# toposware/schnorr-sig

Hardware: AMD Instinct MI355X
Metric: Schnorr verifications/sec, 2^20-sig batch, 1/2/4/8 MI355X; bit-exact vs CPU (higher is better)
Workload: dtype u64

## Files before the change

### __graft_entry__.py

```python
import os
import subprocess
import sys

ROOT = os.path.dirname(os.path.abspath(__file__))
CSRC = os.path.join(ROOT, "schnorr-sig_amd", "csrc")
LIB = os.path.join(CSRC, "libschnorr_sig_amd.so")


def _sources():
    return sorted(f for f in os.listdir(CSRC) if f.endswith((".hip", ".hpp", ".hpp", ".inc")))


STAMP = LIB + ".srchash"


def _source_hash(deps):
    import hashlib
    h = hashlib.sha256()
    for d in sorted(deps):
        h.update(os.path.basename(d).encode() + b"\0")
        with open(d, "rb") as fh:
            h.update(fh.read())
        h.update(b"\0")
    return h.hexdigest()


HIPCC_FLAGS = ["-O3", "--offload-arch=gfx950", "-std=c++17", "-fPIC"]


def _file_sha256(path):
    import hashlib
    h = hashlib.sha256()
    with open(path, "rb") as fh:
        for blk in iter(lambda: fh.read(1 << 20), b""):
            h.update(blk)
    return h.hexdigest()


_TOOLCHAIN = []


def _toolchain():
    if not _TOOLCHAIN:
        try:
            _TOOLCHAIN.append(subprocess.run(["hipcc", "--version"], capture_output=True, text=True, timeout=60).stdout.strip())
        except Exception:
            _TOOLCHAIN.append(None)
    return _TOOLCHAIN[0]


def _stamp(deps):
    return {"sources": _source_hash(deps), "flags": " ".join(HIPCC_FLAGS), "hipcc": _toolchain()}


def _stale(target, deps):
    import json
    if not os.path.exists(target) or not os.path.exists(STAMP):
        return True
    try:
        with open(STAMP) as fh:
            st = json.load(fh)
    except ValueError:
        return True
    want = _stamp(deps)
    if want["hipcc"] is None:
        want.pop("hipcc")
    return any(st.get(k) != v for k, v in want.items()) or st.get("library_sha256") != _file_sha256(target)


def build(force=False):
    params_inc = os.path.join(ROOT, "schnorr-sig_amd", "params", "params_default.inc")
    if not os.path.exists(params_inc):
        subprocess.check_call([sys.executable, os.path.join(ROOT, "schnorr-sig_amd", "params", "gen_params.py")])
    deps = [os.path.join(CSRC, s) for s in _sources()] + [params_inc, os.path.join(ROOT, "include", "schnorr_sig_amd.h")]
    if force or _stale(LIB, deps):
        if _toolchain() is None:
            raise RuntimeError("the HIP library is missing or stale and there is no hipcc on this host to rebuild it")
        objs, procs = [], []
        for unit in ("ssa_api", "ssa_msm", "ssa_sign"):
            objs.append(unit + ".o")
            procs.append(subprocess.Popen(["hipcc"] + HIPCC_FLAGS + ["-c", "-cuid=" + unit, "-o", unit + ".o",
                                           unit + ".hip"], cwd=CSRC))
        for pr in procs:
            if pr.wait() != 0:
                raise subprocess.CalledProcessError(pr.returncode, pr.args)
        subprocess.check_call(["hipcc", "--offload-arch=gfx950", "-fPIC", "-shared", "-o", os.path.basename(LIB)] + objs,
                              cwd=CSRC)
        objs = [os.path.join(CSRC, o) for o in objs]
        for obj in objs:
            os.remove(obj)
        import json
        st = _stamp(deps)
        st["library_sha256"] = _file_sha256(LIB)
        with open(STAMP, "w") as fh:
            json.dump(st, fh, indent=1)
    subprocess.check_call(["make", "-s", "-C", os.path.join(ROOT, "oracle")])
    if ROOT not in sys.path:
        sys.path.insert(0, ROOT)
    import schnorr_sig_amd


def smoke():
    import numpy as np
    if ROOT not in sys.path:
        sys.path.insert(0, ROOT)
    sys.path.insert(0, os.path.join(ROOT, "oracle"))
    import schnorr_sig_amd as ssa
    from oracle import Oracle

    n = 256
    rng = np.random.default_rng(0x5C4E0222)
    sks = rng.integers(0, 256, size=(n, 32), dtype=np.uint8)
    sks[:, 31] &= 0x3F
    nonces = rng.integers(0, 256, size=(n, 32), dtype=np.uint8)
    nonces[:, 31] &= 0x3F
    msgs = rng.integers(0, 256, size=(n, 80), dtype=np.uint8)
    eng = ssa.Engine(0)
    pks, sigs = eng.keygen_sign_many(sks, nonces, msgs)
    orc = Oracle()
    pks_o, sigs_o = orc.keygen_sign_many(sks[:16], nonces[:16], msgs[:16])
    assert (pks[:16] == pks_o).all() and (sigs[:16] == sigs_o).all(), "GPU keygen/sign != oracle"
    sigs[3, 49] ^= 1
    msgs[7, 0] ^= 1
    pks[11] = pks[12]
    status, nfail = eng.verify_many(sigs, pks, msgs, check_torsion=True)
    expect = orc.verify_many(sigs, pks, msgs, check_torsion=True)
    assert (status == expect).all(), "GPU status vector != oracle"
    assert nfail == int((expect != 0).sum()) == 3
    print("smoke ok: %d signatures, %d rejected as expected" % (n, nfail))


if __name__ == "__main__":
    build()
    if len(sys.argv) > 1 and sys.argv[1] == "smoke":
        smoke()
```

### schnorr-sig_amd/csrc/curve.hpp

```cpp
#pragma once
#include "fp6.hpp"

namespace ssa {

struct jac {
    fp6 X, Y, Z;
};
struct aff {
    fp6 x, y;
};

SSA_DEV jac jac_identity() {
    jac r;
    r.X = f6_one();
    r.Y = f6_one();
    r.Z = f6_zero();
    return r;
}
SSA_DEV bool jac_is_identity(const jac &p) { return f6_is_zero(p.Z); }

#ifdef SSA_DBL_PLAIN
SSA_DEV jac jac_dbl(const jac &p) {
    fp6 XX = f6_sqr(p.X);
    fp6 YY = f6_sqr(p.Y);
    fp6 YYYY = f6_sqr(YY);
    fp6 ZZ = f6_sqr(p.Z);
    fp6 t = f6_add(p.X, YY);
    fp6 S = f6_dbl(f6_sub(f6_sub(f6_sqr(t), XX), YYYY));
    fp6 M = f6_add(f6_add(f6_dbl(XX), XX), f6_sqr(ZZ));
    jac r;
    r.X = f6_sub(f6_sqr(M), f6_dbl(S));
    fp6 y8 = f6_dbl(f6_dbl(f6_dbl(YYYY)));
    r.Y = f6_sub(f6_mul(M, f6_sub(S, r.X)), y8);
    fp6 yz = f6_add(p.Y, p.Z);
    r.Z = f6_sub(f6_sub(f6_sqr(yz), YY), ZZ);
    return r;
}
#else
SSA_DEV jac jac_dbl(const jac &p) {
#ifdef SSA_DBL_INLINE
    const fp6 XX = f6_sqr_inl(p.X);
    const fp6 YY = f6_sqr_inl(p.Y);
    const fp6 YYYY = f6_sqr_inl(YY);
    const fp6 ZZ = f6_sqr_inl(p.Z);
#else
    const fp6 XX = f6_sqr(p.X);
    const fp6 YY = f6_sqr(p.Y);
    const fp6 YYYY = f6_sqr(YY);
    const fp6 ZZ = f6_sqr(p.Z);
#endif
    const fp6 Sh = f6_sqr_sub2(f6_add(p.X, YY), XX, YYYY);
    const fp6 M = f6_sqr_add3x(ZZ, XX);
    jac r;
    r.X = f6_sqr_sub4x(M, Sh);
    r.Y = f6_mul_sub8x(M, f6_sub(f6_dbl(Sh), r.X), YYYY);
    r.Z = f6_sqr_sub2(f6_add(p.Y, p.Z), YY, ZZ);
    return r;
}
#endif

#if defined(SSA_F6_ASM) && !defined(SSA_NO_JAC_ASM)
#define SSA_JAC_ASM 1
#ifdef SSA_JAC_ASM_INC
#include SSA_JAC_ASM_INC
#else
#include "jac_asm.inc"
#endif
#endif
SSA_DEV jac jac_dbl_n(jac p, u32 n) {
    if (n == 0) return p;
#ifdef SSA_JAC_ASM
    jac_dbl_n_asm(p.X.c, p.Y.c, p.Z.c, n);
    return p;
#else
#pragma unroll 1
    for (u32 d = 0; d < n; d++) p = jac_dbl(p);
    return p;
#endif
}

SSA_FN void jac_dbl_cold(jac *__restrict__ r, const jac *__restrict__ p) { *r = jac_dbl(*p); }

SSA_DEV jac jac_madd(const jac &p, const aff &q) {
#ifdef SSA_MADD_PLAIN
    fp6 Z1Z1 = f6_sqr(p.Z);
    fp6 U2 = f6_mul(q.x, Z1Z1);
    fp6 S2 = f6_mul(f6_mul(q.y, p.Z), Z1Z1);
    fp6 H = f6_sub(U2, p.X);
    fp6 R = f6_sub(S2, p.Y);
#else
    const fp6 Z1Z1 = f6_sqr(p.Z);
    u64 zz7[6];
    f6_mul_prescale(Z1Z1, zz7);
    const fp6 H = f6_mul_subx_pre(q.x, Z1Z1, zz7, p.X);
    const fp6 R = f6_mul_subx_pre(f6_mul(q.y, p.Z), Z1Z1, zz7, p.Y);
#endif
    const bool p_inf = f6_is_zero(p.Z);
    const bool q_inf = f6_is_zero(q.x) && f6_is_zero(q.y);
    const bool h0 = f6_is_zero(H);
    const bool r0 = f6_is_zero(R);
    if (!p_inf && !q_inf && h0 && r0) {
#ifndef SSA_MADD_COLD_DBL
        return jac_dbl(p);
#else
        jac d;
        jac_dbl_cold(&d, &p);
        return d;
#endif
    }
    fp6 HH = f6_sqr(H);
    fp6 HHH = f6_mul(H, HH);
    fp6 V = f6_mul(p.X, HH);
    jac r;
#ifdef SSA_MADD_PLAIN
    r.X = f6_sub(f6_sub(f6_sqr(R), HHH), f6_dbl(V));
    r.Y = f6_sub(f6_mul(R, f6_sub(V, r.X)), f6_mul(p.Y, HHH));
#else
    r.X = f6_sqr_subx_sub2y(R, HHH, V);
    r.Y = f6_mul2_add(R, f6_sub(V, r.X), f6_neg(p.Y), HHH);
#endif
    r.Z = f6_mul(p.Z, H);
    if (p_inf) {
        r.X = q.x;
        r.Y = q.y;
        r.Z = q_inf ? f6_zero() : f6_one();
    }
    if (q_inf && !p_inf) r = p;
    return r;
}

SSA_DEV jac jac_madd_fast(const jac &p, const aff &q) {
#ifdef SSA_JAC_ASM
    jac r = p;
    if (jac_madd_asm(r.X.c, r.Y.c, r.Z.c, q.x.c, q.y.c)) return r;
    return jac_madd(r, q);
#else
    return jac_madd(p, q);
#endif
}

SSA_DEV jac jac_add(const jac &p, const jac &q) {
    fp6 Z1Z1 = f6_sqr(p.Z);
    fp6 Z2Z2 = f6_sqr(q.Z);
    fp6 U1 = f6_mul(p.X, Z2Z2);
    fp6 U2 = f6_mul(q.X, Z1Z1);
    fp6 S1 = f6_mul(f6_mul(p.Y, q.Z), Z2Z2);
    fp6 S2 = f6_mul(f6_mul(q.Y, p.Z), Z1Z1);
    fp6 H = f6_sub(U2, U1);
    fp6 R = f6_sub(S2, S1);
    const bool p_inf = f6_is_zero(p.Z);
    const bool q_inf = f6_is_zero(q.Z);
    if (!p_inf && !q_inf && f6_is_zero(H) && f6_is_zero(R)) {
#ifndef SSA_MADD_COLD_DBL
        return jac_dbl(p);
#else
        jac d;
        jac_dbl_cold(&d, &p);
        return d;
#endif
    }
    fp6 HH = f6_sqr(H);
    fp6 HHH = f6_mul(H, HH);
    fp6 V = f6_mul(U1, HH);
    jac r;
    r.X = f6_sub(f6_sub(f6_sqr(R), HHH), f6_dbl(V));
    r.Y = f6_sub(f6_mul(R, f6_sub(V, r.X)), f6_mul(S1, HHH));
    r.Z = f6_mul(f6_mul(p.Z, q.Z), H);
    if (p_inf) r = q;
    if (q_inf && !p_inf) r = p;
    return r;
}

SSA_DEV jac jac_neg_if(const jac &p, bool neg) {
    jac r = p;
    fp6 ny = f6_neg(p.Y);
    r.Y = f6_select(neg, p.Y, ny);
    return r;
}

SSA_DEV jac jac_from_aff(const aff &a) {
    jac r;
    r.X = a.x;
    r.Y = a.y;
    r.Z = f6_one();
    return r;
}

SSA_DEV aff jac_to_aff(const jac &p) {
    aff r;
    if (f6_is_zero(p.Z)) {
        r.x = f6_zero();
        r.y = f6_zero();
        return r;
    }
    fp6 zi = f6_inv(p.Z);
    fp6 zi2 = f6_sqr(zi);
    r.x = f6_canon(f6_mul(p.X, zi2));
    r.y = f6_canon(f6_mul(p.Y, f6_mul(zi, zi2)));
    return r;
}

struct sc256 {
    u64 w[4];
};
SSA_DEV u64 sc_q_limb(int i) {
    switch (i) {
        case 0: return 0xd443623eaed4accfULL;
        case 1: return 0x327aa72330157722ULL;
        case 2: return 0x563fbf0f990a37b5ULL;
        default: return 0x7af2599b3b3f22d0ULL;
    }
}
#define SC_Q(i) sc_q_limb(i)

SSA_DEV bool sc_geq_q(const sc256 &a) {
    bool ge = true;
#pragma unroll
    for (int i = 0; i < 4; i++) {
        if (a.w[i] > SC_Q(i)) ge = true;
// ... 95 lines not shown
```

### schnorr-sig_amd/csrc/ssa_kernels.hpp

```cpp
#pragma once
#include "curve.hpp"
#include "fp3.hpp"
#include "rescue.hpp"

namespace ssa {

struct GtabGeom {
    u32 bits, count;
};
constexpr int GW_BITS_MAX = 24, GW_BITS_MIN = 16;
__host__ __device__ inline u32 gtab_windows(u32 bits) { return (255u + bits) / bits; }
__host__ __device__ inline size_t gtab_entries(u32 bits) { return (size_t)gtab_windows(bits) << bits; }
__host__ __device__ inline size_t gbase_entries(u32 bits) { return ((size_t)gtab_windows(bits) * 2) << (bits / 2); }
__host__ __device__ inline u64 gtab_header(u32 bits) { return (u64)bits | ((u64)gtab_windows(bits) << 8); }
SSA_DEV GtabGeom gtab_geom(const u64 *__restrict__ gtab) {
    const u32 v = (u32)__builtin_amdgcn_readfirstlane((int)(u32)gtab[0]);
    GtabGeom g;
    g.bits = v & 0xffu;
    g.count = (v >> 8) & 0xffu;
    return g;
}
constexpr int PTAB_ENTRIES = 16;
constexpr int PTAB_ENTRY_U64 = 32, PTAB_Z = 16, PTAB_C = 22;
constexpr int PTAB_NEG = 16, PTAB_NY = PTAB_NEG + 6;
// ... 209 lines not shown
SSA_DEV void st_row(u64 *__restrict__ row, const jac &p) {
    st_f6(row, p.X);
    st_f6(row + 6, p.Y);
    st_f6(row + PTAB_Z, p.Z);
}
SSA_DEV jac ld_row(const u64 *__restrict__ row) {
    jac p;
    p.X = ld_f6(row);
    p.Y = ld_f6(row + 6);
    p.Z = ld_f6(row + PTAB_Z);
    return p;
}

SSA_FN void tab_dbl(u64 *__restrict__ dst, const u64 *__restrict__ src) { st_row(dst, jac_dbl(ld_row(src))); }
SSA_FN void tab_madd(u64 *__restrict__ dst, const u64 *__restrict__ src, const u64 *__restrict__ paff) {
    st_row(dst, jac_madd(ld_row(src), ld_aff(paff)));
}

SSA_DEV fp6 aff_dbl_num(const fp6 &x) {
    const fp6 xx = f6_sqr(x);
    fp6 n = f6_add(f6_dbl(xx), xx);
    n.c[0] = fp_add(n.c[0], 1ull);
    return n;
}
SSA_DEV aff aff_from_slope(const fp6 &l, const fp6 &x1, const fp6 &y1, const fp6 &x2) {
    aff r;
    r.x = f6_sub(f6_sub(f6_sqr(l), x1), x2);
    r.y = f6_sub(f6_mul(l, f6_sub(x1, r.x)), y1);
    return r;
}
SSA_DEV void st_tab_entry(u64 *__restrict__ row, const aff &a) {
    st_aff(row, a);
    st_f6(row + PTAB_NEG, a.x);
    st_f6(row + PTAB_NY, f6_neg(a.y));
}
SSA_DEV bool build_ptab_affine_upper(u64 *__restrict__ tab) {
    constexpr int R = PTAB_ENTRY_U64;
    const aff p8 = ld_aff(tab + 7 * R);
    fp6 c = f6_one();
#pragma unroll 1
    for (int m = 9; m <= 16; m++) {
        const aff b = ld_aff(tab + (((m & 1) ? m - 8 : m / 2) - 1) * R);
        const fp6 d = (m & 1) ? f6_sub(p8.x, b.x) : f6_dbl(b.y);
        st_f6(tab + (m - 1) * R + PTAB_Z, d);
        c = f6_mul(c, d);
        st_f6(tab + (m - 1) * R + PTAB_C, c);
    }
    if (f6_is_zero(c)) return false;
    fp6 inv = f6_inv(c);
#pragma unroll 1
    for (int m = 16; m >= 9; m--) {
        fp6 di = inv;
        if (m > 9) di = f6_mul(inv, ld_f6(tab + (m - 2) * R + PTAB_C));
        inv = f6_mul(inv, ld_f6(tab + (m - 1) * R + PTAB_Z));
        const aff b = ld_aff(tab + (((m & 1) ? m - 8 : m / 2) - 1) * R);
        aff r;
        if (m & 1) r = aff_from_slope(f6_mul(f6_sub(p8.y, b.y), di), b.x, b.y, p8.x);
        else r = aff_from_slope(f6_mul(aff_dbl_num(b.x), di), b.x, b.y, b.x);
        st_tab_entry(tab + (m - 1) * R, r);
    }
    return true;
}

SSA_DEV bool build_ptab_affine(u64 *__restrict__ tab, const aff &p) {
    constexpr int R = PTAB_ENTRY_U64;
    const fp6 d2 = f6_dbl(p.y);
    if (f6_is_zero(d2)) return false;
    const aff p2 = aff_from_slope(f6_mul(aff_dbl_num(p.x), f6_inv(d2)), p.x, p.y, p.x);
    const fp6 a3 = f6_sub(p2.x, p.x), a4 = f6_dbl(p2.y);
    const fp6 t34 = f6_mul(a3, a4);
    if (f6_is_zero(t34)) return false;
    const fp6 i34 = f6_inv(t34);
    const aff p3 = aff_from_slope(f6_mul(f6_sub(p2.y, p.y), f6_mul(i34, a4)), p.x, p.y, p2.x);
    const aff p4 = aff_from_slope(f6_mul(aff_dbl_num(p2.x), f6_mul(i34, a3)), p2.x, p2.y, p2.x);
    const fp6 a5 = f6_sub(p4.x, p.x), a6 = f6_dbl(p3.y), a7 = f6_sub(p4.x, p3.x), a8 = f6_dbl(p4.y);
    const fp6 t56 = f6_mul(a5, a6), t567 = f6_mul(t56, a7), t5678 = f6_mul(t567, a8);
    if (f6_is_zero(t5678)) return false;
    fp6 inv = f6_inv(t5678);
    const fp6 i8 = f6_mul(inv, t567);
    inv = f6_mul(inv, a8);
    const fp6 i7 = f6_mul(inv, t56);
    inv = f6_mul(inv, a7);
    const fp6 i6 = f6_mul(inv, a5), i5 = f6_mul(inv, a6);
    st_tab_entry(tab, p);
    st_tab_entry(tab + 1 * R, p2);
    st_tab_entry(tab + 2 * R, p3);
    st_tab_entry(tab + 3 * R, p4);
    st_tab_entry(tab + 4 * R, aff_from_slope(f6_mul(f6_sub(p4.y, p.y), i5), p.x, p.y, p4.x));
    st_tab_entry(tab + 5 * R, aff_from_slope(f6_mul(aff_dbl_num(p3.x), i6), p3.x, p3.y, p3.x));
    st_tab_entry(tab + 6 * R, aff_from_slope(f6_mul(f6_sub(p4.y, p3.y), i7), p3.x, p3.y, p4.x));
    st_tab_entry(tab + 7 * R, aff_from_slope(f6_mul(aff_dbl_num(p4.x), i8), p4.x, p4.y, p4.x));
    return build_ptab_affine_upper(tab);
}

SSA_DEV void build_ptab(u64 *__restrict__ tab, const aff &p, bool p_inf) {
    constexpr int R = PTAB_ENTRY_U64;
    if (p_inf) {
        aff z;
        z.x = f6_zero();
        z.y = f6_zero();
#pragma unroll 1
        for (int e = 0; e < PTAB_ENTRIES; e++) st_tab_entry(tab + e * R, z);
        return;
    }
#ifndef SSA_PTAB_JACOBIAN_ONLY
    if (build_ptab_affine(tab, p)) return;
#endif
    st_row(tab, jac_from_aff(p));
    tab_dbl(tab + 1 * R, tab);
    tab_madd(tab + 2 * R, tab + 1 * R, tab);
    tab_dbl(tab + 3 * R, tab + 1 * R);
    tab_madd(tab + 4 * R, tab + 3 * R, tab);
    tab_dbl(tab + 5 * R, tab + 2 * R);
    tab_madd(tab + 6 * R, tab + 5 * R, tab);
    tab_dbl(tab + 7 * R, tab + 3 * R);
#pragma unroll 1
    for (int m = 9; m <= 16; m++) {
        if (m & 1) tab_madd(tab + (m - 1) * R, tab + (m - 2) * R, tab);
        else tab_dbl(tab + (m - 1) * R, tab + (m / 2 - 1) * R);
    }
    fp6 c = f6_one();
#pragma unroll 1
    for (int e = 1; e < PTAB_ENTRIES; e++) {
        fp6 z = ld_f6(tab + e * R + PTAB_Z);
        if (f6_is_zero(z)) z = f6_one();
        c = f6_mul(c, z);
        st_f6(tab + e * R + PTAB_C, c);
    }
    fp6 inv = f6_inv(c);
#pragma unroll 1
    for (int e = PTAB_ENTRIES - 1; e >= 1; e--) {
        fp6 z = ld_f6(tab + e * R + PTAB_Z);
        const bool zero = f6_is_zero(z);
        if (zero) z = f6_one();
        fp6 zinv = inv;
        if (e > 1) zinv = f6_mul(inv, ld_f6(tab + (e - 1) * R + PTAB_C));
        inv = f6_mul(inv, z);
        const fp6 zi2 = f6_sqr(zinv);
        aff a;
        a.x = f6_mul(ld_f6(tab + e * R), zi2);
        a.y = f6_mul(ld_f6(tab + e * R + 6), f6_mul(zi2, zinv));
        if (zero) {
            a.x = f6_zero();
            a.y = f6_zero();
        }
        st_tab_entry(tab + e * R, a);
    }
    st_tab_entry(tab, p);
}

#include "qnaf.inc"

constexpr int LADDER_STEPS = 50, LADDER_STEPS_Q = QNAF_LEN - 1;
SSA_DEV jac ladder_init(const u64 *__restrict__ tab, const sc256 &kr, bool order_q) {
    jac acc = jac_identity();
    const u32 top = order_q ? (u32)QNAF_DIGIT[0] : sc_top5(kr);
    if (top != 0) {
        const aff p = ld_aff(tab + ((top > 16u ? 16u : top) - 1u) * PTAB_ENTRY_U64);
        if (!(f6_is_zero(p.x) && f6_is_zero(p.y))) acc = jac_from_aff(p);
        if (top > 16u) acc = jac_madd_fast(acc, ld_aff(tab + (top - 17u) * PTAB_ENTRY_U64));
    }
    return acc;
}
SSA_DEV jac ladder_steps(jac acc, const u64 *&tab, const sc256 &kr, bool order_q, int lo, int hi) {
#pragma unroll 1
    for (int it = lo; it < hi; it++) {
        int digit;
        u32 gap;
        if (order_q) {
            digit = (int)QNAF_DIGIT[it + 1];
            gap = (u32)QNAF_GAP[it + 1];
        } else {
            digit = (int)sc_win5(kr, (u32)(49 - it)) - 16;
            gap = 5u;
        }
        const int mag = digit < 0 ? -digit : digit;
#ifdef SSA_JAC_ASM
#ifdef SSA_GATHER_HOT
        const u64 *row = tab;
#else
        const u64 *row = tab + (size_t)((mag ? mag : 1) - 1) * PTAB_ENTRY_U64 + (digit < 0 ? PTAB_NEG : 0);
#endif
        if (__builtin_expect(!jac_window_asm(acc.X.c, acc.Y.c, acc.Z.c, row, (u32)mag, gap, tab), 0)) {
            if (digit != 0) {
                aff q;
                q.x = ld_f6(row);
                q.y = ld_f6(row + 6);
                acc = jac_madd(acc, q);
            }
        }
#else
        acc = jac_dbl_n(acc, gap);
        if (digit != 0) {
            aff q = ld_aff(tab + (mag - 1) * PTAB_ENTRY_U64);
            q.y = f6_select(digit < 0, q.y, f6_neg(q.y));
            acc = jac_madd_fast(acc, q);
        }
#endif
    }
    return acc;
}
SSA_DEV jac mul_ptab(const u64 *__restrict__ tab_in, const sc256 &k, bool order_q = false) {
    const sc256 kr = sc_recode_offset5(k);
    const u64 *tab = tab_in;
    return ladder_steps(ladder_init(tab, kr, order_q), tab, kr, order_q, 0, order_q ? LADDER_STEPS_Q : LADDER_STEPS);
}

SSA_DEV jac jac_madd_gather(const jac &p, const u64 *row, const u64 *next, const u64 *&base) {
#ifdef SSA_JAC_ASM
    jac r = p;
    if (__builtin_expect(jac_madd_gather_asm(r.X.c, r.Y.c, r.Z.c, row, next, base) != 0, 1)) return r;
    return jac_madd(r, ld_aff(row));
#else
    (void)next;
    (void)base;
    return jac_madd(p, ld_aff(row));
#endif
}

SSA_DEV jac comb_add(jac acc, const u64 *__restrict__ base_in, const sc256 &k, u32 bits, u32 count, bool hot = false) {
    const u64 *base = base_in;
#pragma unroll 1
    for (u32 w = 0; w < count; w++) {
        const u32 d = sc_bits(k, w * bits, bits);
        if (d != 0) {
            const u32 w1 = w + 1 < count ? w + 1 : w;
            const u64 *next = base + (((size_t)w1 << bits) + sc_bits(k, w1 * bits, bits)) * 12;
#ifdef SSA_COMB_HOT
            const u64 *row = base + (hot ? (size_t)12 : (((size_t)w << bits) + d) * 12);
#else
            const u64 *row = base + (((size_t)w << bits) + d) * 12;
#endif
            acc = jac_madd_gather(acc, row, next, base);
        }
    }
    return acc;
}

SSA_DEV jac add_base_mul(jac acc, const u64 *__restrict__ gtab, const sc256 &e, bool hot = false) {
    const GtabGeom gg = gtab_geom(gtab);
    return comb_add(acc, gtab, e, gg.bits, gg.count, hot);
}

SSA_DEV u32 sig_flag_precheck(u32 flag, bool x_is_zero) {
    if (flag & 0x3fu) return ST_MALFORMED;
    if ((flag & 0x80u) && (!x_is_zero || (flag & 0x40u))) return ST_MALFORMED;
    return ST_OK;
}
SSA_FN bool jac_y_lex_largest(const jac &p) {
    const fp6 zi = f6_inv(p.Z);
    const fp6 y = f6_mul(p.Y, f6_mul(zi, f6_sqr(zi)));
    return f6_lex_largest(y);
}

SSA_FN bool x_on_curve(const fp6 &x) {
    fp6 rhs = f6_add(f6_mul(f6_sqr(x), x), x);
    rhs.c[0] = fp_add(rhs.c[0], 395ull);
    rhs.c[1] = fp_add(rhs.c[1], 1ull);
    return f6_is_square(rhs);
}

constexpr u32 VF_CHECK_TORSION = 1u, VF_SIG_FLAG_BYTE = 8u;
#ifdef SSA_WAVE_TIMES
constexpr size_t SSA_WAVE_TIMES_MAX = 1u << 16;
__device__ unsigned long long g_wave_times[3 * SSA_WAVE_TIMES_MAX];
__device__ unsigned long long g_phase_times[4 * SSA_WAVE_TIMES_MAX];
#define SSA_PHASE_MARK(k) do { if (!in_piece && lane == 0 && (size_t)blockIdx.x * 4u + (threadIdx.x >> 6) < SSA_WAVE_TIMES_MAX) \
    g_phase_times[4 * ((size_t)blockIdx.x * 4u + (threadIdx.x >> 6)) + (k)] = wall_clock64(); } while (0)
#else
#define SSA_PHASE_MARK(k) do { } while (0)
#endif

constexpr int VP_MAX = 8;
struct TailPlan {
    u32 n_pieces;
    u32 tail_groups;
    u32 main_blocks;
    u32 ph[VP_MAX];
    u32 whole[2];
    u32 reversed;
};
__host__ __device__ inline u32 tail_grid_blocks(const TailPlan &tp) { return tp.main_blocks + tp.n_pieces * (tp.tail_groups / 4u); }
struct BlockRole {
    u32 piece;
    u32 index;
};
SSA_DEV BlockRole tail_role(const TailPlan &tp, u32 blk) {
    BlockRole r;
    r.piece = 0xffffffffu;
    r.index = blk;
    if (tp.n_pieces == 0) return r;
    const u32 pb = tp.tail_groups / 4u;
    if (blk < pb) {
        r.piece = 0;
        return r;
    }
    if (blk < pb + tp.main_blocks) {
        r.index = blk - pb;
        return r;
    }
    const u32 q = blk - pb - tp.main_blocks;
    r.piece = 1u + q / pb;
    r.index = q - (r.piece - 1u) * pb;
    return r;
}
constexpr int PARK_WORDS = 19;
SSA_DEV void st_shared(u64 *__restrict__ p, u64 v) { __hip_atomic_store(p, v, __ATOMIC_RELAXED, __HIP_MEMORY_SCOPE_AGENT); }
SSA_DEV void park_store(u64 *__restrict__ pk, const jac &r) {
#pragma unroll
    for (int k = 0; k < 6; k++) {
        st_shared(pk + k * 64, r.X.c[k]);
        st_shared(pk + (6 + k) * 64, r.Y.c[k]);
        st_shared(pk + (12 + k) * 64, r.Z.c[k]);
    }
}
SSA_DEV jac park_load(const u64 *__restrict__ pk) {
    jac r;
#pragma unroll
    for (int k = 0; k < 6; k++) {
        r.X.c[k] = pk[k * 64];
        r.Y.c[k] = pk[(6 + k) * 64];
        r.Z.c[k] = pk[(12 + k) * 64];
    }
    return r;
}

#ifndef SSA_NO_KERNELS
__global__ void __launch_bounds__(256, 2)
ssa_k_verify(const u8 *__restrict__ sigs, const u8 *__restrict__ pks,
             const u8 *__restrict__ pk_inf, const u64 *__restrict__ h_in,
             const u64 *__restrict__ gtab, u64 *__restrict__ ws_tab, size_t n, u32 flags,
             u8 *__restrict__ status_out, unsigned long long *__restrict__ n_fail,
             TailPlan tp, u32 *__restrict__ done, u64 *__restrict__ park) {
#ifdef SSA_WAVE_TIMES
    const unsigned long long wt0 = wall_clock64();
#endif
    const BlockRole role = tail_role(tp, tp.reversed ? gridDim.x - 1u - blockIdx.x : blockIdx.x);
    const u32 lane = threadIdx.x & 63u;
    const bool in_piece = role.piece != 0xffffffffu;
    const u32 p_lo = in_piece ? role.piece : 0u;
    const u32 eg = in_piece ? 4u * role.index + (threadIdx.x >> 6) : 0u;
    const size_t i = in_piece ? ((size_t)tp.main_blocks * 256u + (size_t)eg * 64u + lane)
                              : ((size_t)role.index * blockDim.x + threadIdx.x);
    const bool runs_last = !in_piece || p_lo + 1u == tp.n_pieces;
    const bool in = i < n;
    u64 *pk = park + ((size_t)eg * PARK_WORDS) * 64 + lane;
    u64 *tab = ws_tab + i * (size_t)(PTAB_ENTRIES * PTAB_ENTRY_U64);
    u32 status = ST_OK;
    bool ok_sig = true;
    jac r = jac_identity();
    u32 run_lo = p_lo;
    if (in_piece) {
        u32 *next = done + tp.tail_groups + eg;
        u32 cur = 0;
        if (lane == 0) {
            cur = __hip_atomic_load(next, __ATOMIC_RELAXED, __HIP_MEMORY_SCOPE_AGENT);
            while (cur <= p_lo) {
                const u32 seen = atomicCAS(next, cur, p_lo + 1u);
                if (seen == cur) break;
                cur = seen;
            }
        }
        cur = (u32)__builtin_amdgcn_readfirstlane((int)cur);
        if (cur > p_lo) return;
        run_lo = cur;
    }
    if (in_piece && run_lo > 0) {
        while (__hip_atomic_load(done + eg, __ATOMIC_RELAXED, __HIP_MEMORY_SCOPE_AGENT) < run_lo) __builtin_amdgcn_s_sleep(64);
        __builtin_amdgcn_fence(__ATOMIC_ACQUIRE, "agent");
        asm volatile("s_waitcnt vmcnt(0)" ::: "memory");
        const u64 sw = pk[18 * 64];
        status = (u32)(sw & 0xffu);
        ok_sig = ((sw >> 8) & 1u) != 0;
        if (in && status == ST_OK && !(tp.ph[run_lo] & 2u)) r = park_load(pk);
    } else if (in) {
        bool ok = true;
        const fp6 xs = ld_fp6(sigs + 81 * i, ok_sig);
        const sc256 e = ld_sc(sigs + 81 * i + 49);
        ok_sig = ok_sig && !sc_geq_q(e);
        const u32 fbyte = sigs[81 * i + 48];
        if ((flags & VF_SIG_FLAG_BYTE) && ok_sig) ok_sig = sig_flag_precheck(fbyte, f6_is_zero(xs)) == ST_OK;
        aff P;
        P.x = ld_fp6(pks + 96 * i, ok);
        P.y = ld_fp6(pks + 96 * i + 48, ok);
        const bool inf = pk_inf && pk_inf[i];
        if (ok && !inf) ok = aff_on_curve(P);
        if (!ok) status = ST_MALFORMED;
        else build_ptab(tab, P, inf);
    }
    SSA_PHASE_MARK(1);
    if (in && status == ST_OK) {
        sc256 h;
#pragma unroll
        for (int k = 0; k < 4; k++) h.w[k] = h_in[4 * i + k];
        const sc256 kr = sc_recode_offset5(h);
        const u32 d_lo = in_piece ? run_lo : ((flags & VF_CHECK_TORSION) ? 0u : 1u);
        const u32 d_hi = in_piece ? p_lo + 1u : 2u;
        const u64 *ltab = tab;
#pragma unroll 1
        for (u32 k = d_lo; k < d_hi; k++) {
            const u32 d = in_piece ? tp.ph[k] : tp.whole[k];
            const bool pass_q = (d & 1u) == 0, first = (d & 2u) != 0, last = (d & 4u) != 0;
            if (first) {
                if (!pass_q && !ok_sig) {
                    status = ST_MALFORMED;
                    break;
                }
                r = ladder_init(ltab, kr, pass_q);
            }
            r = ladder_steps(r, ltab, kr, pass_q, (int)((d >> 8) & 0xffu), (int)((d >> 16) & 0xffu));
            if (last && pass_q && !jac_is_identity(r)) {
                status = ST_INVALID_PK;
                break;
            }
        }
    }
    SSA_PHASE_MARK(2);
    if (runs_last) {
        if (in) {
            if (status == ST_OK) {
                bool okx = true;
                const fp6 xs = ld_fp6(sigs + 81 * i, okx);
                const sc256 e = ld_sc(sigs + 81 * i + 49);
                const u32 fbyte = sigs[81 * i + 48];
#ifdef SSA_COMB_HOT
                r = add_base_mul(r, gtab, e, true);
#else
                r = add_base_mul(r, gtab, e);
#endif
                bool eq;
                if (flags & VF_SIG_FLAG_BYTE) {
                    if (fbyte & 0x80u) {
                        eq = jac_is_identity(r);
                    } else {
                        eq = !jac_is_identity(r) && f6_eq(r.X, f6_mul(xs, f6_sqr(r.Z)));
                        if (eq) eq = jac_y_lex_largest(r) == ((fbyte & 0x40u) != 0);
#ifndef SSA_COMB_HOT
                        else if (!x_on_curve(xs)) ok_sig = false;
#endif
                    }
                } else if (jac_is_identity(r)) {
                    eq = f6_is_zero(xs);
                } else {
                    eq = f6_eq(r.X, f6_mul(xs, f6_sqr(r.Z)));
                }
                status = eq ? ST_OK : (ok_sig ? ST_INVALID_SIG : ST_MALFORMED);
            }
            status_out[i] = (u8)status;
        }
        const unsigned long long bad = __ballot(status != ST_OK);
        if (lane == 0 && bad) atomicAdd(n_fail, (unsigned long long)__popcll(bad));
    } else {
        if (in && status == ST_OK) park_store(pk, r);
        st_shared(pk + 18 * 64, (u64)status | ((u64)(ok_sig ? 1u : 0u) << 8));
        asm volatile("s_waitcnt vmcnt(0)" ::: "memory");
        if (run_lo == 0) {
            __builtin_amdgcn_fence(__ATOMIC_RELEASE, "agent");
            asm volatile("s_waitcnt vmcnt(0)" ::: "memory");
        }
        __hip_atomic_store(done + eg, p_lo + 1u, __ATOMIC_RELAXED, __HIP_MEMORY_SCOPE_AGENT);
    }
#ifdef SSA_WAVE_TIMES
    SSA_PHASE_MARK(3);
    if (lane == 0) {
        const size_t w = (size_t)blockIdx.x * (blockDim.x / 64u) + (threadIdx.x >> 6);
        if (w < SSA_WAVE_TIMES_MAX) {
            if (!in_piece) g_phase_times[4 * w] = wt0;
            g_wave_times[3 * w] = wt0;
            g_wave_times[3 * w + 1] = wall_clock64();
            g_wave_times[3 * w + 2] = ((unsigned long long)__builtin_amdgcn_s_getreg((20 << 0) | (0 << 6) | (31 << 11)) << 32) |
                                      (unsigned long long)__builtin_amdgcn_s_getreg((4 << 0) | (0 << 6) | (31 << 11));
        }
    }
#endif
}
#endif

#ifndef SSA_NO_KERNELS
__global__ void __launch_bounds__(256, 2)
ssa_k_keyset_build(const u8 *__restrict__ pks, const u8 *__restrict__ pk_inf, size_t m, u64 *__restrict__ key_tab,
                   u8 *__restrict__ key_status) {
    const size_t i = (size_t)blockIdx.x * blockDim.x + threadIdx.x;
    if (i >= m) return;
    bool ok = true;
    aff P;
    P.x = ld_fp6(pks + 96 * i, ok);
    P.y = ld_fp6(pks + 96 * i + 48, ok);
    const bool inf = pk_inf && pk_inf[i];
    if (ok && !inf) ok = aff_on_curve(P);
    u32 st = ST_MALFORMED;
    if (ok) {
        u64 *tab = key_tab + i * (size_t)(PTAB_ENTRIES * PTAB_ENTRY_U64);
        build_ptab(tab, P, inf);
        sc256 q;
#pragma unroll
        for (int j = 0; j < 4; j++) q.w[j] = SC_Q(j);
        st = jac_is_identity(mul_ptab(tab, q, true)) ? ST_OK : ST_INVALID_PK;
    }
    key_status[i] = (u8)st;
}

__global__ void __launch_bounds__(256, 2)
ssa_k_verify_keyed(const u8 *__restrict__ sigs, const u32 *__restrict__ key_idx, const u64 *__restrict__ key_tab,
                   const u8 *__restrict__ key_status, u32 n_keys, const u64 *__restrict__ h_in,
                   const u64 *__restrict__ gtab, size_t n, u32 flags, u8 *__restrict__ status_out,
                   unsigned long long *__restrict__ n_fail) {
    const size_t i = (size_t)blockIdx.x * blockDim.x + threadIdx.x;
    u32 status = ST_OK;
    if (i < n) {
        bool ok_sig = true;
        const fp6 xs = ld_fp6(sigs + 81 * i, ok_sig);
        const sc256 e = ld_sc(sigs + 81 * i + 49);
        ok_sig = ok_sig && !sc_geq_q(e);
        const u32 fbyte = sigs[81 * i + 48];
        if ((flags & VF_SIG_FLAG_BYTE) && ok_sig) ok_sig = sig_flag_precheck(fbyte, f6_is_zero(xs)) == ST_OK;
        const u32 k = key_idx[i];
        const u32 ks = k < n_keys ? (u32)key_status[k] : ST_MALFORMED;
        if (ks == ST_MALFORMED) status = ST_MALFORMED;
        else if (ks == ST_INVALID_PK && (flags & VF_CHECK_TORSION)) status = ST_INVALID_PK;
        else if (!ok_sig) status = ST_MALFORMED;
        if (status == ST_OK) {
            const u64 *tab = key_tab + (size_t)k * (size_t)(PTAB_ENTRIES * PTAB_ENTRY_U64);
            sc256 h;
#pragma unroll
            for (int j = 0; j < 4; j++) h.w[j] = h_in[4 * i + j];
            jac r = mul_ptab(tab, h);
            r = add_base_mul(r, gtab, e);
            bool eq;
            if (flags & VF_SIG_FLAG_BYTE) {
                if (fbyte & 0x80u) {
                    eq = jac_is_identity(r);
                } else {
                    eq = !jac_is_identity(r) && f6_eq(r.X, f6_mul(xs, f6_sqr(r.Z)));
                    if (eq) eq = jac_y_lex_largest(r) == ((fbyte & 0x40u) != 0);
                    else if (!x_on_curve(xs)) ok_sig = false;
                }
            } else if (jac_is_identity(r)) {
                eq = f6_is_zero(xs);
            } else {
                eq = f6_eq(r.X, f6_mul(xs, f6_sqr(r.Z)));
            }
            status = eq ? ST_OK : (ok_sig ? ST_INVALID_SIG : ST_MALFORMED);
        }
        status_out[i] = (u8)status;
    }
    const unsigned long long bad = __ballot(status != ST_OK);
    if ((threadIdx.x & 63u) == 0 && bad) atomicAdd(n_fail, (unsigned long long)__popcll(bad));
}
#endif

constexpr int KB_BITS = 8, KB_COUNT = 32;
constexpr size_t KBASE_ENTRIES_PER_KEY = (size_t)KB_COUNT << KB_BITS;
constexpr int KW_BITS = 16, KW_COUNT = 16;
constexpr size_t KTAB_ENTRIES_PER_KEY = (size_t)KW_COUNT << KW_BITS;

#ifndef SSA_NO_KERNELS
__global__ void __launch_bounds__(256)
ssa_k_keycomb_base(const u8 *__restrict__ pks, const u8 *__restrict__ pk_inf, const u8 *__restrict__ key_status,
                    size_t m, u64 *__restrict__ kbase) {
    const size_t t = (size_t)blockIdx.x * blockDim.x + threadIdx.x;
    if (t >= m * KBASE_ENTRIES_PER_KEY) return;
    const size_t key = t / KBASE_ENTRIES_PER_KEY;
    const u32 w = (u32)((t >> KB_BITS) % KB_COUNT), d = (u32)(t & ((1u << KB_BITS) - 1u));
    aff a;
    a.x = f6_zero();
    a.y = f6_zero();
    const bool inf = pk_inf && pk_inf[key];
    if (key_status[key] != ST_MALFORMED && !inf && d != 0) {
        bool ok = true;
        aff P;
        P.x = ld_fp6(pks + 96 * key, ok);
        P.y = ld_fp6(pks + 96 * key + 48, ok);
        jac acc = jac_identity();
#pragma unroll 1
        for (int b = KB_BITS - 1; b >= 0; b--) {
            acc = jac_dbl(acc);
            if ((d >> b) & 1u) acc = jac_madd(acc, P);
        }
#pragma unroll 1
        for (u32 k = 0; k < w * KB_BITS; k++) acc = jac_dbl(acc);
        a = jac_to_aff(acc);
    }
    ulonglong2 *q = reinterpret_cast<ulonglong2 *>(kbase + t * 12);
#pragma unroll
    for (int i = 0; i < 3; i++) {
        q[i] = make_ulonglong2(a.x.c[2 * i], a.x.c[2 * i + 1]);
        q[3 + i] = make_ulonglong2(a.y.c[2 * i], a.y.c[2 * i + 1]);
    }
}

__global__ void __launch_bounds__(256)
ssa_k_keycomb_build(const u64 *__restrict__ kbase, size_t m, u64 *__restrict__ ktab) {
    const size_t t = (size_t)blockIdx.x * blockDim.x + threadIdx.x;
    if (t >= m * (KTAB_ENTRIES_PER_KEY / 8)) return;
    const size_t key = t / (KTAB_ENTRIES_PER_KEY / 8), e0 = (t % (KTAB_ENTRIES_PER_KEY / 8)) * 8;
    const u32 w = (u32)(e0 >> KW_BITS), d0 = (u32)(e0 & ((1u << KW_BITS) - 1u));
    const u32 dhi = d0 >> KB_BITS, dlo0 = d0 & ((1u << KB_BITS) - 1u);
    const u64 *kb = kbase + key * KBASE_ENTRIES_PER_KEY * 12;
    const u64 *slo = kb + ((size_t)(2 * w) << KB_BITS) * 12, *shi = kb + ((size_t)(2 * w + 1) << KB_BITS) * 12;
    u64 *out = ktab + (key * KTAB_ENTRIES_PER_KEY + e0) * 12;
    const aff p1 = ld_aff(shi + (size_t)dhi * 12);
    const bool p1_inf = f6_is_zero(p1.x) && f6_is_zero(p1.y);
    if (p1_inf) {
#pragma unroll 1
        for (int k = 0; k < 8; k++) st_aff(out + 12 * k, ld_aff(slo + (size_t)(dlo0 + k) * 12));
        return;
    }
// ... 749 lines not shown
```

Measured before the change: 30.68 million.

## Use sign-flipped Jacobian window asm with lazy negation and LDS-cached scalar windows

Replaces the per-window Jacobian step with a generated 'sign-flip' assembly routine. The accumulator may be kept in negated form, tracked per lane as a ballot mask and carried through parked state, with a single conditional negation at the end. The recoded scalar is stored in LDS so 5-bit windows can be read with shifts instead of recomputed from registers. The top-digit second addition is folded into the ladder as a step at index -1. This aims to shorten the double-and-add sequence, but it adds a build-time code generator and more complex sign bookkeeping that must stay bit-exact.

```diff
diff --git a/__graft_entry__.py b/__graft_entry__.py
--- a/__graft_entry__.py
+++ b/__graft_entry__.py
@@ -68,7 +68,27 @@
     return any(st.get(k) != v for k, v in want.items()) or st.get("library_sha256") != _file_sha256(target)
 
 
+def _generate_sf():
+    import importlib.util
+    import io
+    from contextlib import redirect_stdout
+    spec = importlib.util.spec_from_file_location("gen_jac_asm", os.path.join(ROOT, "tools", "gen_jac_asm.py"))
+    mod = importlib.util.module_from_spec(spec)
+    spec.loader.exec_module(mod)
+    with redirect_stdout(io.StringIO()):
+        text = mod.generate_sf()
+    try:
+        with open(mod.OUT_PATH_SF) as fh:
+            if fh.read() == text:
+                return
+    except OSError:
+        pass
+    with open(mod.OUT_PATH_SF, "w") as fh:
+        fh.write(text)
+
+
 def build(force=False):
+    _generate_sf()
     params_inc = os.path.join(ROOT, "schnorr-sig_amd", "params", "params_default.inc")
     if not os.path.exists(params_inc):
         subprocess.check_call([sys.executable, os.path.join(ROOT, "schnorr-sig_amd", "params", "gen_params.py")])
diff --git a/schnorr-sig_amd/csrc/curve.hpp b/schnorr-sig_amd/csrc/curve.hpp
--- a/schnorr-sig_amd/csrc/curve.hpp
+++ b/schnorr-sig_amd/csrc/curve.hpp
@@ -65,6 +65,11 @@
 #include SSA_JAC_ASM_INC
 #else
 #include "jac_asm.inc"
+#endif
+#ifdef SSA_JAC_SF_ASM_INC
+#include SSA_JAC_SF_ASM_INC
+#else
+#include "jac_sf_asm.inc"
 #endif
 #endif
 SSA_DEV jac jac_dbl_n(jac p, u32 n) {
diff --git a/schnorr-sig_amd/csrc/ssa_kernels.hpp b/schnorr-sig_amd/csrc/ssa_kernels.hpp
--- a/schnorr-sig_amd/csrc/ssa_kernels.hpp
+++ b/schnorr-sig_amd/csrc/ssa_kernels.hpp
@@ -385,45 +385,92 @@
 #include "qnaf.inc"
 
 constexpr int LADDER_STEPS = 50, LADDER_STEPS_Q = QNAF_LEN - 1;
-SSA_DEV jac ladder_init(const u64 *__restrict__ tab, const sc256 &kr, bool order_q) {
+#ifdef SSA_JAC_ASM
+#define SSA_LADDER_LDS 1
+SSA_DEV u64 *ladder_words() {
+    __shared__ u64 kr_sh[4 * 256];
+    return kr_sh + (threadIdx.x & 255u);
+}
+#endif
+SSA_DEV void ladder_scalar(const sc256 &kr) {
+#ifdef SSA_LADDER_LDS
+    u64 *w = ladder_words();
+#pragma unroll
+    for (int k = 0; k < 4; k++) w[k * 256] = kr.w[k];
+#else
+    (void)kr;
+#endif
+}
+SSA_DEV u32 ladder_win5(const sc256 &kr, u32 w) {
+#ifdef SSA_LADDER_LDS
+    (void)kr;
+    const u64 *p = ladder_words();
+    const u32 bit = 5u * w, wi = bit >> 6, sh = bit & 63u;
+    u64 v = p[wi * 256u] >> sh;
+    if (sh > 59u) v |= p[(wi + 1u) * 256u] << (64u - sh);
+    return (u32)v & 31u;
+#else
+    return sc_win5(kr, w);
+#endif
+}
+SSA_DEV u32 ladder_top(const sc256 &kr, bool order_q) {
+    if (order_q) return (u32)QNAF_DIGIT[0];
+#ifdef SSA_LADDER_LDS
+    (void)kr;
+    return (u32)(ladder_words()[3 * 256] >> 58);
+#else
+    return sc_top5(kr);
+#endif
+}
+SSA_DEV jac ladder_init(const u64 *__restrict__ tab, const sc256 &kr, bool order_q, u32 &form) {
     jac acc = jac_identity();
-    const u32 top = order_q ? (u32)QNAF_DIGIT[0] : sc_top5(kr);
+    form = 0;
+    const u32 top = ladder_top(kr, order_q);
     if (top != 0) {
         const aff p = ld_aff(tab + ((top > 16u ? 16u : top) - 1u) * PTAB_ENTRY_U64);
         if (!(f6_is_zero(p.x) && f6_is_zero(p.y))) acc = jac_from_aff(p);
-        if (top > 16u) acc = jac_madd_fast(acc, ld_aff(tab + (top - 17u) * PTAB_ENTRY_U64));
     }
     return acc;
 }
-SSA_DEV jac ladder_steps(jac acc, const u64 *&tab, const sc256 &kr, bool order_q, int lo, int hi) {
+SSA_DEV jac ladder_steps(jac acc, const u64 *&tab, const sc256 &kr, bool order_q, int lo, int hi, u32 &form) {
+#ifdef SSA_JAC_ASM
+    u64 fm = __ballot(form != 0);
+#endif
 #pragma unroll 1
     for (int it = lo; it < hi; it++) {
         int digit;
         u32 gap;
-        if (order_q) {
+        if (it < 0) {
+            const u32 top = ladder_top(kr, order_q);
+            digit = top > 16u ? (int)top - 16 : 0;
+            gap = 0u;
+        } else if (order_q) {
             digit = (int)QNAF_DIGIT[it + 1];
             gap = (u32)QNAF_GAP[it + 1];
         } else {
-            digit = (int)sc_win5(kr, (u32)(49 - it)) - 16;
+            digit = (int)ladder_win5(kr, (u32)(49 - it)) - 16;
             gap = 5u;
         }
         const int mag = digit < 0 ? -digit : digit;
 #ifdef SSA_JAC_ASM
+        const bool want_neg = __builtin_amdgcn_inverse_ballot_w64(~(__ballot(digit < 0) ^ fm));
 #ifdef SSA_GATHER_HOT
         const u64 *row = tab;
 #else
-        const u64 *row = tab + (size_t)((mag ? mag : 1) - 1) * PTAB_ENTRY_U64 + (digit < 0 ? PTAB_NEG : 0);
-#endif
-        if (__builtin_expect(!jac_window_asm(acc.X.c, acc.Y.c, acc.Z.c, row, (u32)mag, gap, tab), 0)) {
+        const u64 *row = tab + (size_t)((mag ? mag : 1) - 1) * PTAB_ENTRY_U64 + (want_neg ? PTAB_NEG : 0);
+#endif
+        const bool done = jac_window_sf_asm(acc.X.c, acc.Y.c, acc.Z.c, row, (u32)mag, gap, tab) != 0;
+        fm ^= __ballot(done && mag != 0);
+        if (__builtin_expect(!done, 0)) {
             if (digit != 0) {
                 aff q;
                 q.x = ld_f6(row);
-                q.y = ld_f6(row + 6);
+                q.y = ld_f6(want_neg ? row + 6 - PTAB_NEG : row + PTAB_NY);
                 acc = jac_madd(acc, q);
             }
         }
 #else
-        acc = jac_dbl_n(acc, gap);
+        if (gap) acc = jac_dbl_n(acc, gap);
         if (digit != 0) {
             aff q = ld_aff(tab + (mag - 1) * PTAB_ENTRY_U64);
             q.y = f6_select(digit < 0, q.y, f6_neg(q.y));
@@ -431,12 +478,18 @@
         }
 #endif
     }
+#ifdef SSA_JAC_ASM
+    form = __builtin_amdgcn_inverse_ballot_w64(fm) ? 1u : 0u;
+#endif
     return acc;
 }
 SSA_DEV jac mul_ptab(const u64 *__restrict__ tab_in, const sc256 &k, bool order_q = false) {
     const sc256 kr = sc_recode_offset5(k);
     const u64 *tab = tab_in;
-    return ladder_steps(ladder_init(tab, kr, order_q), tab, kr, order_q, 0, order_q ? LADDER_STEPS_Q : LADDER_STEPS);
+    u32 form;
+    ladder_scalar(kr);
+    const jac acc = ladder_init(tab, kr, order_q, form);
+    return jac_neg_if(ladder_steps(acc, tab, kr, order_q, -1, order_q ? LADDER_STEPS_Q : LADDER_STEPS, form), form != 0);
 }
 
 SSA_DEV jac jac_madd_gather(const jac &p, const u64 *row, const u64 *next, const u64 *&base) {
@@ -582,6 +635,7 @@
     u32 status = ST_OK;
     bool ok_sig = true;
     jac r = jac_identity();
+    u32 form = 0;
     u32 run_lo = p_lo;
     if (in_piece) {
         u32 *next = done + tp.tail_groups + eg;
@@ -605,6 +659,7 @@
         const u64 sw = pk[18 * 64];
         status = (u32)(sw & 0xffu);
         ok_sig = ((sw >> 8) & 1u) != 0;
+        form = (u32)(sw >> 9) & 1u;
         if (in && status == ST_OK && !(tp.ph[run_lo] & 2u)) r = park_load(pk);
     } else if (in) {
         bool ok = true;
@@ -627,6 +682,7 @@
 #pragma unroll
         for (int k = 0; k < 4; k++) h.w[k] = h_in[4 * i + k];
         const sc256 kr = sc_recode_offset5(h);
+        ladder_scalar(kr);
         const u32 d_lo = in_piece ? run_lo : ((flags & VF_CHECK_TORSION) ? 0u : 1u);
         const u32 d_hi = in_piece ? p_lo + 1u : 2u;
         const u64 *ltab = tab;
@@ -639,9 +695,9 @@
                     status = ST_MALFORMED;
                     break;
                 }
-                r = ladder_init(ltab, kr, pass_q);
+                r = ladder_init(ltab, kr, pass_q, form);
             }
-            r = ladder_steps(r, ltab, kr, pass_q, (int)((d >> 8) & 0xffu), (int)((d >> 16) & 0xffu));
+            r = ladder_steps(r, ltab, kr, pass_q, first ? -1 : (int)((d >> 8) & 0xffu), (int)((d >> 16) & 0xffu), form);
             if (last && pass_q && !jac_is_identity(r)) {
                 status = ST_INVALID_PK;
                 break;
@@ -656,6 +712,7 @@
                 const fp6 xs = ld_fp6(sigs + 81 * i, okx);
                 const sc256 e = ld_sc(sigs + 81 * i + 49);
                 const u32 fbyte = sigs[81 * i + 48];
+                r = jac_neg_if(r, form != 0);
 #ifdef SSA_COMB_HOT
                 r = add_base_mul(r, gtab, e, true);
 #else
@@ -685,7 +742,7 @@
         if (lane == 0 && bad) atomicAdd(n_fail, (unsigned long long)__popcll(bad));
     } else {
         if (in && status == ST_OK) park_store(pk, r);
-        st_shared(pk + 18 * 64, (u64)status | ((u64)(ok_sig ? 1u : 0u) << 8));
+        st_shared(pk + 18 * 64, (u64)status | ((u64)(ok_sig ? 1u : 0u) << 8) | ((u64)form << 9));
         asm volatile("s_waitcnt vmcnt(0)" ::: "memory");
         if (run_lo == 0) {
             __builtin_amdgcn_fence(__ATOMIC_RELEASE, "agent");
```

New measurement: 30.78 million, median of 6. No clear change (+0.3%).
